# iKrishneel/fcn_object_detector

Measured on AMD Instinct MI355X. Metric: frames/sec forward 448x448 @1 GPU; train imgs/sec @1/2/4/8 GPUs, higher is better.
Workload: dtype f32; 1 GPU; configs[1]: single-GPU forward, DetectNet GoogLeNet conv stack + coverage/bbox heads (graph of models/deploy.prototxt), batch=1, 448x448, random-init weights; global_batch=1, parallelism=replicas x1, frames_in_flight=4

## Files before the change

### fcn_object_detector_amd/engine.py

```python
from __future__ import annotations

import ctypes as C
import os
import threading
from collections import namedtuple
from dataclasses import dataclass, field
from typing import Callable, Dict, List, Optional, Sequence, Tuple, Union

import numpy as np

from . import lib as L
from . import storage as S
from . import tune as T
from .netspec import Layer, NetSpec, bn_global_stats, crop_window, interp_size, is_rectangular, kernel_stride_pad, layer_dilation, layer_geometry
from .storage import _r4, _ra, ip_pack_bank, ip_unpack_bank

F32 = np.float32


def graphs_enabled() -> bool:
    return os.environ.get("FCN_NO_GRAPH", "0") in ("", "0")


_replica_ctx = threading.local()
# ... 74 lines not shown
    @property
    def bytes(self) -> float:
        return 4.0 * (self.n * self.cin * self.h * self.w + self.n * self.cout * self.oh * self.ow + self.cout * self.cin * self.kh * self.kw + self.cout)

    def swapped(self) -> "RectGeom":
        return self._replace(cin=self.cout, h=self.oh, w=self.ow, cout=self.cin, oh=self.h, ow=self.w)


def rconv_desc(x: "Blob", y: "Blob", g: RectGeom, w: Optional[int] = None, bias: Optional[int] = None, flags: int = 0) -> L.RConvDesc:
    d = L.RConvDesc()
    d.x, d.w, d.bias, d.y = x.ptr, w, bias, y.buf.ptr
    d.N, d.H, d.W, d.Cin, d.x_cstride = g.n, g.h, g.w, g.cin, x.cstride
    d.Cout, d.kh, d.kw, d.pad_h, d.pad_w, d.stride_h, d.stride_w, d.OH, d.OW = g.cout, g.kh, g.kw, g.ph, g.pw, g.sh, g.sw, g.oh, g.ow
    d.y_cstride, d.y_coffset = y.cstride, y.coffset
    d.flags, d.dilation = flags, g.d
    return d


class DwGeom(namedtuple("DwGeom", "n c h w oh ow kh kw sh sw ph pw d")):
    __slots__ = ()

    @property
    def flops(self) -> float:
        return 2.0 * self.n * self.oh * self.ow * self.c * self.kh * self.kw

    @property
    def bytes(self) -> float:
        return 4.0 * (self.n * self.h * self.w * self.c + self.n * self.oh * self.ow * self.c + self.kh * self.kw * self.c + self.c)


# ... 158 lines not shown
    return ranges_hit(later.reads, earlier.writes) or ranges_hit(later.writes, earlier.writes) or ranges_hit(later.writes, earlier.reads)


def task_levels(tasks: Sequence[Task], group_convs: bool = True) -> List[int]:
    levels: List[int] = []
    for i, ti in enumerate(tasks):
        levels.append(max([levels[j] + 1 for j in range(i) if task_waits(ti, tasks[j])], default=0) if group_convs else i)
    return levels


def task_floats(tasks: Sequence[Task], levels: Sequence[int], i: int) -> bool:
    return not any(levels[j] == levels[i] + 1 and task_waits(tj, tasks[i]) for j, tj in enumerate(tasks) if j != i)


class Engine:

    def __init__(self, spec: NetSpec, data_shapes: Optional[Dict[str, Tuple[int, ...]]] = None,
                 params: Optional[Dict[str, List[np.ndarray]]] = None, device: int = 0,
                 fuse: bool = True, group_convs: bool = True, autotune: bool = True, dtype: str = "f32",
                 tune_from: Optional["Engine"] = None, tune_max_lds_kb: Optional[int] = None,
                 share_params: Optional["Engine"] = None, score_outputs: bool = False, replica: Optional[int] = None):
        if dtype not in ("f32", "f16"):
            raise ValueError("dtype must be 'f32' or 'f16'")
        if share_params is not None and (dtype != "f32" or share_params.f16):
            raise NotImplementedError("share_params: only between float32 engines (a half-float engine packs its weights differently)")
        self._share_from = share_params
        self.shared_layers: set = set()
        self.score_outputs = bool(score_outputs)
        self.score_acc: Dict[str, DeviceBuffer] = {}
        self.graph_score: Optional[int] = None
# ... 16 lines not shown
        yes = C.c_int(0)
        L.call("fcn_stream_is_prioritized", self.stream, C.byref(yes))
        self.stream_prioritized = bool(yes.value)
        self.lock = threading.RLock()
        self.shapes = spec.infer(data_shapes)
        self.blobs: Dict[str, Blob] = {}
        self.params_host: Dict[str, List[np.ndarray]] = {}
        self.params_dev: Dict[str, List[DevView]] = {}
        self.ops: List[Op] = []
        self.graph_io: Optional[int] = None
        self.graph_core: Optional[int] = None
        self._staging: Dict[str, DeviceBuffer] = {}
        self._keep: List[object] = []
        self._conv_layer_meta: Dict[str, dict] = {}
        self._group_workspaces: List[DeviceBuffer] = []
        self.aux_dev: Dict[str, DeviceBuffer] = {}
        self._bn_chains: Dict[str, BnChain] = {}
        self._bn_ws_bytes = 0
        self._bn_ws: Optional[DeviceBuffer] = None
        self._lazy_blob_ops: Dict[str, List[Op]] = {}
        self.loss_blobs: Dict[str, float] = {}
        self.device_fed: set = set()
        self.dropout_seed = 0
        self.dropout_index_offset = 0
        self.inputs = spec.data_tops()
        self.outputs = [b for b in spec.output_blobs() if b in self.shapes]
        max_lds = int(tune_max_lds_kb if tune_max_lds_kb is not None else os.environ.get("FCN_TUNE_MAX_LDS_KB", "160")) * 1024
        self.tuner = T.Tuner(self.stream, T.key_suffix(self.shapes.get(self.inputs[0], ()) if self.inputs else None, self.f16, max_lds),
                             spec.phase == "TEST", max_lds, tune_from._chosen_cfgs if tune_from is not None else None)
        self._plan_buffers()
# ... 63 lines not shown
            self.param_segs[(seg.layer, seg.index)] = seg
            self.params_dev.setdefault(seg.layer, []).append(DevView(self.param_flat.ptr + 4 * seg.offset, seg.nbytes))
        for l in self.spec.param_layers():
            if l.name not in self.shared_layers:
                self._upload_params(l)

    def _folded_shift(self, l: Layer) -> float:
        return next((sh for t, sh in self._half_inputs.values() if t == l.bottoms[0]), 0.0) if l.type == "Convolution" else 0.0

    def _upload_params(self, l: Layer) -> None:
        if l.name in self.shared_layers:
            raise RuntimeError("layer %s reads the parameters of another engine (share_params): set them there" % l.name)
        packed = [S.pack(self.param_segs[(l.name, i)], h, self._folded_shift(l) if i == 0 else 0.0) for i, h in enumerate(self.params_host[l.name])]
        for arr, dev in zip(packed, self.params_dev[l.name]):
            L.call("fcn_memcpy_h2d_async", dev.ptr, arr.ctypes.data, arr.nbytes, None)
        L.call("fcn_device_sync")

    def set_params(self, layer: str, blobs: Sequence[np.ndarray]) -> None:
        lay = next(l for l in self.spec.layers if l.name == layer)
        if layer in self.shared_layers:
            raise RuntimeError("layer %s reads the parameters of another engine (share_params): set them there" % layer)
        shapes = self.spec.param_shapes[layer]
        self.params_host[layer] = [np.ascontiguousarray(b, dtype=F32).reshape(s).copy() for b, s in zip(blobs, shapes)]
        self._upload_params(lay)

    def read_param(self, layer: str, index: int) -> np.ndarray:
        with self.lock:
            v = self.params_dev[layer][index]
            raw = np.empty(v.nbytes, np.uint8)
            L.call("fcn_memcpy_d2h_async", raw.ctypes.data, v.ptr, raw.nbytes, self.stream)
# ... 218 lines not shown
            read = l.bottoms[:1] if t == "Crop" else l.bottoms
            tasks.append(OpTask(l, ops, reads=[self._range(b) for b in read], writes=[self._range(tp) for tp in l.tops],
                                pool_desc=self._fusable_pool_desc(l)))
        return tasks

    def _build_ops(self) -> None:
        tasks = self._collect_tasks()
        if self._bn_ws_bytes:
            self._bn_ws = DeviceBuffer(self._bn_ws_bytes, zero=False)
        if self.fuse and self.spec.phase == "TEST" and os.environ.get("FCN_FUSE_POOL_LRN", "1") != "0":
            tasks = self._fuse_pool_lrn(tasks)
        levels = task_levels(tasks, self.group_convs)
        if self.autotune and self.group_convs and self.fuse and not self.f16 and self.spec.phase == "TEST" and os.environ.get("FCN_LEVEL_MOVE", "1") != "0":
            self.tuner.move_floaters(tasks, levels)
        tail = self._plan_tail(tasks, levels)
        order = sorted(range(len(tasks)), key=lambda i: (levels[i], 1 if isinstance(tasks[i], ConvTask) else 0, i))
        pending: List[ConvTask] = []
        pending_pools: List[OpTask] = []
        pending_dconvs: List[OpTask] = []
        pending_rconvs: List[OpTask] = []
        cur = None
        for i in order:
            if levels[i] != cur:
                self._emit_dconvs(pending_dconvs)
                self._emit_rconvs(pending_rconvs)
                self._emit_convs(pending, pending_pools, tail)
                pending, pending_dconvs, pending_rconvs, cur = [], [], [], levels[i]
            if tail is not None and any(tasks[i] is ht for ht in tail["heads"]):
                continue
            if isinstance(tasks[i], ConvTask):
                pending.append(tasks[i])
            elif tasks[i].pool_desc is not None and self.fuse and self.group_convs:
                pending_pools.append(tasks[i])
            elif tasks[i].dconv is not None:
                pending_dconvs.append(tasks[i])
            elif tasks[i].rconv is not None:
                pending_rconvs.append(tasks[i])
            else:
                self.ops.extend(tasks[i].ops)
        self._emit_dconvs(pending_dconvs)
        self._emit_rconvs(pending_rconvs)
        self._emit_convs(pending, pending_pools, tail)
        self.levels = max(levels) + 1 if levels else 0
        if self.score_outputs:
            self._emit_score_ops()

    def _dconv_task(self, li: int, l: Layer, skip: set) -> OpTask:
        dil = layer_dilation(l)
        if self.f16:
            raise NotImplementedError("f16 engine: Convolution %s with dilation %d has no half-float kernel" % (l.name, dil))
        if self._conv_groups(l) > 1:
            raise NotImplementedError("Convolution %s: group %d together with dilation %d" % (l.name, self._conv_groups(l), dil))
        g = self._geom(l)
        xb, yb = self.blobs[l.bottoms[0]], self.blobs[l.tops[0]]
        if xb.coffset % 4 or xb.cstride % 4:
            raise NotImplementedError("dilated Convolution %s: input view is not 16-byte aligned" % l.name)
        relu = self._relu_after(li, l, skip)
        self._conv_layer_meta[l.name] = dict(relu=relu, sigmoid_top=None)
        pd = self.params_dev[l.name]
        d = dconv_desc(xb, yb, g, dil, pd[0].ptr, pd[1].ptr if len(pd) > 1 else None, L.CONV_RELU if relu else 0)
# ... 997 lines not shown
            for ws in getattr(self, "_group_workspaces", []):
                if ws.ptr:
                    lib.fcn_conv2d_group_release(ws.ptr)
                    ws.free()
            self._group_workspaces = []
            self.ops = []
            self.tuner.release()

    def __del__(self):
        try:
            self.close()
        except Exception:
            pass


class ForwardPipeline:

    def __init__(self, make_spec: Callable[[], NetSpec], params: Optional[Dict[str, List[np.ndarray]]] = None, device: int = 0, depth: int = 4,
                 max_lds_kb: Optional[int] = 36, **engine_kw):
        if depth < 1:
            raise ValueError("depth must be at least 1")
        self.engines: List[Engine] = []
        if os.environ.get("FCN_PIPE_LDS_KB"):
            max_lds_kb = int(os.environ["FCN_PIPE_LDS_KB"]) or None
        if max_lds_kb is not None:
            engine_kw.setdefault("tune_max_lds_kb", max_lds_kb)
        for i in range(depth):
            self.engines.append(Engine(make_spec(), params=params, device=device, tune_from=self.engines[0] if i else None, replica=i,
                                       **engine_kw))
        self._pending: List[Engine] = []
        self._next = 0

    @property
    def depth(self) -> int:
        return len(self.engines)

    def submit(self, inputs: Dict[str, np.ndarray]) -> None:
        if len(self._pending) >= len(self.engines):
            raise RuntimeError("ForwardPipeline: %d frames already in flight, collect() one first" % len(self._pending))
        eng = self.engines[self._next]
        self._next = (self._next + 1) % len(self.engines)
        for nm, arr in inputs.items():
            eng.host_array(nm)[...] = arr
        eng.forward_begin()
        self._pending.append(eng)

# ... 74 lines not shown
```

### fcn_object_detector_amd/lib.py

```python
from __future__ import annotations

import ctypes as C
import os
import threading
from typing import Optional

_HERE = os.path.dirname(os.path.abspath(__file__))
LIB_PATH = os.environ.get("FCN_LIB_PATH") or os.path.join(_HERE, "libfcnhip.so")


class FcnLibraryError(RuntimeError):
    pass


class FcnError(RuntimeError):
    def __init__(self, code: int, msg: str):
        super().__init__("libfcnhip error %d: %s" % (code, msg))
        self.code = code


class ConvDesc(C.Structure):
    _fields_ = [
        ("x", C.c_void_p), ("w", C.c_void_p), ("bias", C.c_void_p), ("y", C.c_void_p), ("y2", C.c_void_p),
        ("N", C.c_int32), ("H", C.c_int32), ("W", C.c_int32), ("Cin", C.c_int32), ("x_cstride", C.c_int32),
# ... 44 lines not shown
                ("total_tiles", C.c_int32)]


class RConvDesc(C.Structure):
    _fields_ = [
        ("x", C.c_void_p), ("w", C.c_void_p), ("bias", C.c_void_p), ("y", C.c_void_p), ("y2", C.c_void_p),
        ("N", C.c_int32), ("H", C.c_int32), ("W", C.c_int32), ("Cin", C.c_int32), ("x_cstride", C.c_int32),
        ("Cout", C.c_int32), ("kh", C.c_int32), ("kw", C.c_int32), ("pad_h", C.c_int32), ("pad_w", C.c_int32),
        ("stride_h", C.c_int32), ("stride_w", C.c_int32), ("OH", C.c_int32), ("OW", C.c_int32),
        ("y_cstride", C.c_int32), ("y_coffset", C.c_int32), ("y2_cstride", C.c_int32), ("y2_coffset", C.c_int32),
        ("flags", C.c_int32), ("dilation", C.c_int32),
    ]


class RConvPlan(C.Structure):
    _fields_ = [("d_probs", C.c_void_p), ("n", C.c_int32), ("cfg", C.c_int32), ("grid_x", C.c_int32), ("grid_y", C.c_int32),
                ("total_tiles", C.c_int32)]


class DwConvDesc(C.Structure):
    _fields_ = [
        ("x", C.c_void_p), ("w", C.c_void_p), ("bias", C.c_void_p), ("y", C.c_void_p), ("y2", C.c_void_p),
        ("N", C.c_int32), ("H", C.c_int32), ("W", C.c_int32), ("C", C.c_int32), ("x_cstride", C.c_int32),
        ("kh", C.c_int32), ("kw", C.c_int32), ("pad_h", C.c_int32), ("pad_w", C.c_int32),
        ("stride_h", C.c_int32), ("stride_w", C.c_int32), ("OH", C.c_int32), ("OW", C.c_int32),
        ("y_cstride", C.c_int32), ("y_coffset", C.c_int32), ("y2_cstride", C.c_int32), ("y2_coffset", C.c_int32),
        ("flags", C.c_int32), ("dilation", C.c_int32),
    ]


# ... 190 lines not shown
    "fcn_tconv_bank_floats": (_sz, [_i, _i, _i, _i]),
    "fcn_tconv_bank_pack_f32": (_i, [_vp, _vp, _i, _i, _i, _i, _i, _vp]),
    "fcn_channel_sum_f32": (_i, [_vp, _vp, _i, _i, _i, _i, _vp]),
    "fcn_dconv2d_num_configs": (_i, []),
    "fcn_dconv2d_workspace_bytes": (_sz, [C.POINTER(DConvDesc), _i]),
    "fcn_dconv2d_prepare": (_i, [C.POINTER(DConvDesc), _i, _vp, _i, C.POINTER(DConvPlan)]),
    "fcn_dconv2d_f32": (_i, [C.POINTER(DConvPlan), _vp]),
    "fcn_dconv2d_wgrad_workspace_floats": (_sz, [C.POINTER(DConvDesc)]),
    "fcn_dconv2d_wgrad_f32": (_i, [C.POINTER(DConvDesc), _vp, _vp, _vp, _vp]),
    "fcn_rconv2d_num_configs": (_i, []),
    "fcn_rconv2d_workspace_bytes": (_sz, [C.POINTER(RConvDesc), _i]),
    "fcn_rconv2d_prepare": (_i, [C.POINTER(RConvDesc), _i, _vp, _i, C.POINTER(RConvPlan)]),
    "fcn_rconv2d_f32": (_i, [C.POINTER(RConvPlan), _vp]),
    "fcn_rconv2d_wgrad_workspace_floats": (_sz, [C.POINTER(RConvDesc)]),
    "fcn_rconv2d_wgrad_f32": (_i, [C.POINTER(RConvDesc), _vp, _vp, _vp, _vp]),
    "fcn_dwconv2d_num_configs": (_i, []),
    "fcn_dwconv2d_fwd_f32": (_i, [C.POINTER(DwConvDesc), _i, _vp]),
    "fcn_dwconv2d_fwd_f16": (_i, [C.POINTER(DwConvDesc), _i, _vp]),
    "fcn_dwconv2d_dgrad_f32": (_i, [C.POINTER(DwConvDesc), _i, _vp]),
    "fcn_dwconv2d_wgrad_workspace_floats": (_sz, [C.POINTER(DwConvDesc), _i]),
    "fcn_dwconv2d_wgrad_f32": (_i, [C.POINTER(DwConvDesc), _vp, _vp, _vp, _i, _vp]),
    "fcn_crop_fwd_f32": (_i, [_vp, _vp] + [_i] * 12 + [_vp]),
    "fcn_crop_fwd_f16": (_i, [_vp, _vp] + [_i] * 12 + [_vp]),
    "fcn_crop_bwd_f32": (_i, [_vp, _vp] + [_i] * 13 + [_vp]),
    "fcn_interp_fwd_f32": (_i, [_vp, _vp] + [_i] * 12 + [_vp]),
    "fcn_interp_fwd_f16": (_i, [_vp, _vp] + [_i] * 13 + [_vp]),
    "fcn_interp_bwd_f32": (_i, [_vp, _vp] + [_i] * 13 + [_vp]),
    "fcn_inner_product_workspace_bytes": (_sz, [_i, _i, _i]),
    "fcn_inner_product_fwd_workspace_bytes": (_sz, [_i, _i, _i, _i]),
    "fcn_inner_product_fwd_f32": (_i, [_vp, _i, _vp, _vp, _vp] + [_i] * 6 + [_vp, _vp]),
# ... 72 lines not shown
```

### fcn_object_detector_amd/storage.py

```python
from __future__ import annotations

from dataclasses import dataclass
from typing import Dict, List, Optional, Sequence, Set, Tuple

import numpy as np

from .netspec import Layer, NetSpec, as_nchw

F32 = np.float32


def _r4(c: int) -> int:
    return (c + 3) // 4 * 4


def _ra(c: int, esize: int) -> int:
    eps = 16 // esize
    return (c + eps - 1) // eps * eps


def blob_nchw(shape: Sequence[int], rows: bool) -> Optional[Tuple[int, int, int, int]]:
    if rows and len(shape) == 1:
        return (shape[0], 1, 1, 1)
    return as_nchw(shape)
# ... 217 lines not shown
                elif f16:
                    raise NotImplementedError("f16 engine: layer type Deconvolution with group 1 (%s) has no half-float kernel" % l.name)
                else:
                    kind, shape = DECONV, (c, kh, kw, _r4(cog))
            elif i == 0 and l.type not in ("BatchNorm", "Scale"):
                raise NotImplementedError(l.type)
            count = int(np.prod(shape))
            lr, decay = float(l.lr_mult[i] if i < len(l.lr_mult) else 1.0), float(l.decay_mult[i] if i < len(l.decay_mult) else 1.0)
            if l.type == "BatchNorm":
                lr = decay = 0.0
            segs.append(ParamSeg(l.name, i, kind, off, count, shape, host_shape, lr, decay, count * esize, esize, bottom))
            off += _r4((count * esize + 3) // 4)
    return segs, off


def conv_groups(l: Layer, cout: int, cin_g: int, esize: int) -> int:
    g = int(l.sub("convolution_param").get("group", 1))
    if g == 1:
        return 1
    eps = 16 // esize
    if g < 1 or cout % g:
        raise ValueError("Convolution %s: group %d does not divide num_output %d" % (l.name, g, cout))
    if cin_g % eps or (cout // g) % eps:
        raise NotImplementedError("grouped Convolution %s: group %d leaves %d input and %d output channels per group, not whole 16-byte "
                                  "segments (%d %s)%s" % (l.name, g, cin_g, cout // g, eps, "floats" if esize == 4 else "halves",
                                                          ": depthwise convolution has no kernel here for a NetSpec built without "
                                                          "depthwise=True (caffe.Net and the solvers pass it; type DepthwiseConvolution "
                                                          "needs no keyword)" if cin_g == 1 else ""))
    return g

# ... 45 lines not shown
```

### fcn_object_detector_amd/train.py

```python
from __future__ import annotations

import ctypes as C
import os
import math
from typing import Callable, Dict, List, Optional, Sequence, Tuple

import numpy as np

from . import lib as L
from . import proto
from . import storage as S
from .backward import BackwardPlanner
from .engine import Blob, DevView, DeviceBuffer, Engine, Op, PinnedArray, _r4, graphs_enabled
from .netspec import DATA_TYPES, Layer, NetSpec

F32 = np.float32


class SolverParams:

    KINDS = ("SGD", "NESTEROV", "ADAGRAD", "RMSPROP", "ADADELTA", "ADAM")
    POLICIES = ("fixed", "step", "exp", "inv", "multistep", "poly", "sigmoid")

    def __init__(self, msg: Optional[proto.Msg] = None, **kw):
# ... 79 lines not shown
            return b
        if p == "step":
            return b * self.gamma ** (it // self.stepsize)
        if p == "exp":
            return b * self.gamma ** it
        if p == "inv":
            return b * (1.0 + self.gamma * it) ** (-self.power)
        if p == "multistep":
            return b * self.gamma ** sum(1 for v in self.stepvalue if v <= it)
        if p == "poly":
            return b * (1.0 - float(it) / self.max_iter) ** self.power
        return b / (1.0 + math.exp(-self.gamma * (it - self.stepsize)))


class TrainEngine(Engine):

    def __init__(self, spec: NetSpec, data_shapes: Dict[str, Tuple[int, ...]], params=None, device: int = 0,
                 solver: Optional[SolverParams] = None, comm=None, autotune: bool = True):
        if spec.phase != "TRAIN":
            raise ValueError("TrainEngine needs a TRAIN-phase NetSpec")
        self.solver = solver or SolverParams()
        self.comm = comm
        self.grad_blobs: Dict[str, Blob] = {}
        self.bwd_ops: List[Op] = []
        self.iter = 0
        super().__init__(spec, data_shapes, params, device, fuse=True, group_convs=True, autotune=autotune)
        self._alloc_solver_state()
        self._build_backward()

    def _learns(self, l: Layer) -> bool:
# ... 452 lines not shown
```

### fcn_object_detector_amd/tune.py

```python
from __future__ import annotations

import ctypes as C
import json
import os
from typing import Callable, Dict, Iterable, List, NamedTuple, Optional, Sequence, Tuple

import numpy as np

from . import engine as E
from . import lib as L


def lower_quartile(samples: Sequence[float]) -> float:
    return float(np.percentile(samples, 25))


class Protocol(NamedTuple):
    warm: int
    reps: int
    evict: bool
    samples: int
    stat: Callable[[Sequence[float]], float]
    contenders: int
    margin: float
# ... 182 lines not shown
                return memo[sub]

            best, best_ms = None, 1e30
            for labels in set_partitions(n):
                ms = sum(cost(tuple(i for i in range(n) if labels[i] == g)) for g in sorted(set(labels)))
                if ms < best_ms - 1e-7:
                    best, best_ms = labels, ms
            return "".join(str(g) for g in best)

        choice = self.choose("cut|" + self.key("+".join(it.layer.name for it in chunk)), valid, search)
        groups: Dict[str, List[E.ConvTask]] = {}
        for it, g in zip(chunk, choice):
            groups.setdefault(g, []).append(it)
        return [groups[g] for g in sorted(groups)]

    def move_floaters(self, tasks: Sequence[object], levels: List[int]) -> None:
        for lv in range(max(levels, default=-1)):
            a_idx, b_idx = ([i for i, t in enumerate(tasks) if levels[i] == l2 and isinstance(t, E.ConvTask)] for l2 in (lv, lv + 1))
            if len(a_idx) < 2 or not b_idx or len(a_idx) > 8:
                continue
            fl = [i for i in a_idx if E.task_floats(tasks, levels, i)]
            if not fl or len(fl) > 3 or len(b_idx) + len(fl) > 8:
                continue

            def valid(code) -> bool:
                return isinstance(code, str) and len(code) == len(fl) and set(code) <= {"0", "1"} and (len(fl) < len(a_idx) or "0" in code)

            def search() -> str:
                pools = {l2: [t.pool_desc for j, t in enumerate(tasks) if levels[j] == l2 and isinstance(t, E.OpTask) and t.pool_desc is not None][:2]
                         for l2 in (lv, lv + 1)}
# ... 28 lines not shown
```

### include/fcnhip.h

```cpp
#ifndef FCNHIP_H_
#define FCNHIP_H_

#include <stddef.h>
#include <stdint.h>

#ifdef __cplusplus
extern "C" {
#endif

#define FCN_ABI_VERSION 1

#define FCN_E_ARG       1
#define FCN_E_ALIGN     2
#define FCN_E_UNSUPPORTED 3
#define FCN_E_STATE     4
#define FCN_E_CAPACITY  5

typedef void* fcn_stream_t;
typedef void* fcn_event_t;
typedef void* fcn_graph_t;
typedef void* fcn_comm_t;

int  fcn_abi_version(void);
const char* fcn_last_error_string(void);
// ... 344 lines not shown
} fcn_rconv_desc;
typedef struct fcn_rconv_plan {
    void*   d_probs;
    int32_t n;
    int32_t cfg;
    int32_t grid_x, grid_y;
    int32_t total_tiles;
} fcn_rconv_plan;
int    fcn_rconv2d_num_configs(void);
size_t fcn_rconv2d_workspace_bytes(const fcn_rconv_desc* h_descs, int n);
int    fcn_rconv2d_prepare(const fcn_rconv_desc* h_descs, int n, void* d_workspace, int cfg_request, fcn_rconv_plan* h_out);
int    fcn_rconv2d_f32(const fcn_rconv_plan* h_plan, fcn_stream_t s);
size_t fcn_rconv2d_wgrad_workspace_floats(const fcn_rconv_desc* h_d);
int    fcn_rconv2d_wgrad_f32(const fcn_rconv_desc* h_d, float* dw, float* db, float* d_workspace, fcn_stream_t s);

typedef struct fcn_dwconv_desc {
    void*        x;
    const float* w;
    const float* bias;
    void*        y;
    float*       y2;
    int32_t N, H, W, C, x_cstride;
    int32_t kh, kw, pad_h, pad_w, stride_h, stride_w, OH, OW;
    int32_t y_cstride, y_coffset, y2_cstride, y2_coffset;
    int32_t flags;
    int32_t dilation;
} fcn_dwconv_desc;
int    fcn_dwconv2d_num_configs(void);
int    fcn_dwconv2d_fwd_f32(const fcn_dwconv_desc* h_d, int cfg_request, fcn_stream_t s);
int    fcn_dwconv2d_fwd_f16(const fcn_dwconv_desc* h_d, int cfg_request, fcn_stream_t s);
// ... 58 lines not shown
```

Before: 4576 frames/s.

## Add Winograd F(2x2,3x3) MFMA conv kernel for eligible inference 3x3 convs

Adds a Winograd F(2,3) convolution kernel for stride-1, pad-1 3x3 float32 convolutions. The input transform is done in-register with DPP lane permutes, the 16 transformed-domain GEMMs run on f32 MFMA, and the output transform plus bias and ReLU are fused into the epilogue. Filter banks are pre-transformed on the host when weights are uploaded. Placement is decided per layer by timing the layer with and without the Winograd kernel, and a multi-replica 'flight' mode is also tuned; the path is limited to inference. The aim is fewer multiplies on the 3x3 convolutions, at the cost of extra filter memory, tuning time and slightly different float rounding.

```diff
diff --git a/fcn_object_detector_amd/csrc/wconv.hip b/fcn_object_detector_amd/csrc/wconv.hip
--- /dev/null
+++ b/fcn_object_detector_amd/csrc/wconv.hip
@@ -0,0 +1,298 @@
+#include "conv_common.h"
+
+#include <vector>
+
+namespace fcn {
+namespace {
+
+constexpr int WC_TILES = 32;
+constexpr int WC_BN = 32;
+constexpr int WC_BK = 8;
+constexpr int WC_POS = 16;
+constexpr int WC_THREADS = 256;
+constexpr int WC_STAGE = WC_POS * 32 * WC_BK;
+constexpr int WC_CONFIGS = 1;
+
+struct WConvP {
+    const float* x;
+    const float* u;
+    const float* bias;
+    float* y;
+    int N, H, W, Cin, x_cstride, Cout, OH, OW, y_cstride, y_coffset, flags;
+    int TH, TW, tiles, nblk_n, nchunk;
+    unsigned tw_magic, th_magic;
+};
+
+template <int S0, int S1, int S2, int S3>
+__device__ __forceinline__ float quad_perm(float v) {
+    return __builtin_bit_cast(float, __builtin_amdgcn_update_dpp(0, __builtin_bit_cast(int, v), S0 | (S1 << 2) | (S2 << 4) | (S3 << 6), 0xf, 0xf, false));
+}
+
+__global__ __launch_bounds__(WC_THREADS) void wconv_f32_kernel(const WConvP* __restrict__ probs) {
+    const WConvP& p = probs[blockIdx.z];
+    const int tblk = blockIdx.x, nblk = blockIdx.y;
+    if (tblk * WC_TILES >= p.tiles || nblk >= p.nblk_n) return;
+
+    __shared__ __attribute__((aligned(16))) float smem[4 * WC_STAGE];
+    float* const sV = smem;
+    float* const sU = smem + 2 * WC_STAGE;
+
+    const int tid = threadIdx.x, lane = tid & 63, wave = tid >> 6;
+    const int lj = tid & 3, lq = (tid >> 2) & 1, lt = tid >> 3;
+    int l_off[4] = {0, 0, 0, 0};
+    bool l_ok[4] = {false, false, false, false};
+    {
+        const int t = tblk * WC_TILES + lt;
+        if (t < p.tiles) {
+            const int q = fast_div(t, p.tw_magic), tx = t - q * p.TW;
+            const int n = fast_div(q, p.th_magic), ty = q - n * p.TH;
+            const int ix = 2 * tx - 1 + lj;
+#pragma unroll
+            for (int i = 0; i < 4; ++i) {
+                const int iy = 2 * ty - 1 + i;
+                l_ok[i] = (unsigned)ix < (unsigned)p.W && (unsigned)iy < (unsigned)p.H;
+                l_off[i] = l_ok[i] ? ((n * p.H + iy) * p.W + ix) * p.x_cstride : 0;
+            }
+        }
+    }
+    const float* const ubase = p.u + (size_t)nblk * p.nchunk * WC_STAGE + tid * 4;
+    const int sign_q = lj == 1 ? 0 : (int)0x80000000u;
+
+    v4f regX[4], regU[4];
+    auto fetch = [&](int c) {
+        const float* us = ubase + (size_t)c * WC_STAGE;
+#pragma unroll
+        for (int r = 0; r < 4; ++r) regU[r] = *(const v4f*)(us + r * (WC_THREADS * 4));
+        const int ci = c * WC_BK + lq * 4;
+#pragma unroll
+        for (int i = 0; i < 4; ++i) {
+            regX[i] = v4f{0.f, 0.f, 0.f, 0.f};
+            if (l_ok[i] && ci < p.Cin) {
+                regX[i] = *(const v4f*)(p.x + l_off[i] + ci);
+                if (ci + 1 >= p.Cin) regX[i][1] = 0.f;
+                if (ci + 2 >= p.Cin) regX[i][2] = 0.f;
+                if (ci + 3 >= p.Cin) regX[i][3] = 0.f;
+            }
+        }
+    };
+    auto stage = [&](int buf) {
+        float* dv = sV + buf * WC_STAGE + ((lt + lj) & 31) * WC_BK + lq * 4;
+        float* du = sU + buf * WC_STAGE + tid * 4;
+#pragma unroll
+        for (int r = 0; r < 4; ++r) *(v4f*)(du + r * (WC_THREADS * 4)) = regU[r];
+        v4f t[4];
+        t[0] = regX[0] - regX[2];
+        t[1] = regX[1] + regX[2];
+        t[2] = regX[2] - regX[1];
+        t[3] = regX[1] - regX[3];
+#pragma unroll
+        for (int i = 0; i < 4; ++i) {
+            v4f v;
+#pragma unroll
+            for (int e = 0; e < 4; ++e) {
+                const float a = quad_perm<0, 1, 2, 1>(t[i][e]);
+                const float b = quad_perm<2, 2, 1, 3>(t[i][e]);
+                v[e] = a + __builtin_bit_cast(float, __builtin_bit_cast(int, b) ^ sign_q);
+            }
+            *(v4f*)(dv + (i * 4 + lj) * (32 * WC_BK)) = v;
+        }
+    };
+
+    const int fr = lane & 31, fh = lane >> 5;
+    const int frag = (wave * 4 * 32 + fr) * WC_BK + fh * 4;
+    int fragv[4];
+#pragma unroll
+    for (int pp = 0; pp < 4; ++pp) fragv[pp] = ((wave * 4 + pp) * 32 + ((fr + pp) & 31)) * WC_BK + fh * 4;
+    f32x16 acc[4];
+#pragma unroll
+    for (int pp = 0; pp < 4; ++pp)
+#pragma unroll
+        for (int e = 0; e < 16; ++e) acc[pp][e] = 0.f;
+
+    fetch(0);
+#pragma unroll 1
+    for (int it = 0; it < p.nchunk; ++it) {
+        const int buf = it & 1;
+        stage(buf);
+        if (it + 1 < p.nchunk) fetch(it + 1);
+        __syncthreads();
+        v4f uf[4], vf[4];
+#pragma unroll
+        for (int pp = 0; pp < 4; ++pp) {
+            uf[pp] = *(const v4f*)(sU + buf * WC_STAGE + frag + pp * (32 * WC_BK));
+            vf[pp] = *(const v4f*)(sV + buf * WC_STAGE + fragv[pp]);
+        }
+#pragma unroll
+        for (int e = 0; e < 4; ++e)
+#pragma unroll
+            for (int pp = 0; pp < 4; ++pp) acc[pp] = __builtin_amdgcn_mfma_f32_32x32x2f32(uf[pp][e], vf[pp][e], acc[pp], 0, 0, 0);
+    }
+
+    __syncthreads();
+#pragma unroll
+    for (int pp = 0; pp < 4; ++pp)
+#pragma unroll
+        for (int r = 0; r < 16; ++r)
+            smem[((wave * 4 + pp) * 32 + (r & 3) + 8 * (r >> 2) + 4 * fh) * 32 + fr] = acc[pp][r];
+    __syncthreads();
+
+    const int et = tid & 31, eq = tid >> 5;
+    const int t = tblk * WC_TILES + et;
+    const int co = nblk * WC_BN + eq * 4;
+    if (t >= p.tiles || co >= p.Cout) return;
+    v4f s[2][4];
+#pragma unroll
+    for (int j = 0; j < 4; ++j)
+#pragma unroll
+        for (int e = 0; e < 4; ++e) {
+            const float m0 = smem[((0 * 4 + j) * 32 + eq * 4 + e) * 32 + et], m1 = smem[((1 * 4 + j) * 32 + eq * 4 + e) * 32 + et];
+            const float m2 = smem[((2 * 4 + j) * 32 + eq * 4 + e) * 32 + et], m3 = smem[((3 * 4 + j) * 32 + eq * 4 + e) * 32 + et];
+            s[0][j][e] = (m0 + m1) + m2;
+            s[1][j][e] = (m1 - m2) - m3;
+        }
+    const int q = fast_div(t, p.tw_magic), tx = t - q * p.TW;
+    const int n = fast_div(q, p.th_magic), ty = q - n * p.TH;
+    const bool do_relu = (p.flags & FCN_CONV_RELU) != 0;
+    const bool vec_ok = ((p.y_cstride | p.y_coffset) & 3) == 0 && ((unsigned)(size_t)p.y & 15) == 0 && co + 3 < p.Cout;
+    v4f b4 = {0.f, 0.f, 0.f, 0.f};
+    if (p.bias)
+#pragma unroll
+        for (int e = 0; e < 4; ++e)
+            if (co + e < p.Cout) b4[e] = p.bias[co + e];
+#pragma unroll
+    for (int dy = 0; dy < 2; ++dy)
+#pragma unroll
+        for (int dx = 0; dx < 2; ++dx) {
+            const int oy = 2 * ty + dy, ox = 2 * tx + dx;
+            if (oy >= p.OH || ox >= p.OW) continue;
+            v4f v = dx == 0 ? (s[dy][0] + s[dy][1]) + s[dy][2] : (s[dy][1] - s[dy][2]) - s[dy][3];
+            v += b4;
+            if (do_relu)
+#pragma unroll
+                for (int e = 0; e < 4; ++e) v[e] = fmaxf(v[e], 0.f);
+            float* dst = p.y + (size_t)((n * p.OH + oy) * p.OW + ox) * p.y_cstride + p.y_coffset + co;
+            if (vec_ok) {
+                *(v4f*)dst = v;
+            } else {
+#pragma unroll
+                for (int e = 0; e < 4; ++e)
+                    if (co + e < p.Cout) dst[e] = v[e];
+            }
+        }
+}
+
+int validate(const fcn_wconv_desc& d) {
+    FCN_REQUIRE(d.x && d.y && d.u, FCN_E_ARG, "wconv: null x/u/y");
+    FCN_REQUIRE(d.N > 0 && d.H > 0 && d.W > 0 && d.Cin > 0 && d.Cout > 0, FCN_E_ARG, "wconv: non-positive extent");
+    FCN_REQUIRE(d.kh == 3 && d.kw == 3, FCN_E_UNSUPPORTED, "wconv: kernel window %dx%d is not 3x3", d.kh, d.kw);
+    FCN_REQUIRE(d.stride_h == 1 && d.stride_w == 1, FCN_E_UNSUPPORTED, "wconv: stride %dx%d is not 1", d.stride_h, d.stride_w);
+    FCN_REQUIRE(d.pad_h == 1 && d.pad_w == 1, FCN_E_UNSUPPORTED, "wconv: pad %dx%d is not 1", d.pad_h, d.pad_w);
+    FCN_REQUIRE(d.dilation == 1, FCN_E_UNSUPPORTED, "wconv: dilation %d is not 1", d.dilation);
+    FCN_REQUIRE((d.flags & ~FCN_CONV_RELU) == 0, FCN_E_UNSUPPORTED,
+                "wconv: flags 0x%x outside FCN_CONV_RELU (float32 only; no FCN_CONV_F16 / SIGMOID2 / ACCUM / MASK)", d.flags);
+    FCN_REQUIRE(d.Cin % 4 == 0, FCN_E_ALIGN, "wconv: Cin (%d) must be a multiple of 4", d.Cin);
+    FCN_REQUIRE(d.x_cstride % 4 == 0 && d.x_cstride >= d.Cin, FCN_E_ALIGN, "wconv: x_cstride (%d) must be a multiple of 4 holding Cin (%d)", d.x_cstride,
+                d.Cin);
+    FCN_REQUIRE(((uintptr_t)d.x & 15) == 0 && ((uintptr_t)d.u & 15) == 0, FCN_E_ALIGN, "wconv: x / u must be 16-byte aligned");
+    FCN_REQUIRE(((uintptr_t)d.y & 3) == 0 && (!d.bias || ((uintptr_t)d.bias & 3) == 0), FCN_E_ALIGN, "wconv: y / bias must be 4-byte aligned");
+    FCN_REQUIRE(d.OH == d.H && d.OW == d.W, FCN_E_ARG, "wconv: OH/OW (%d,%d) is not H/W (%d,%d)", d.OH, d.OW, d.H, d.W);
+    FCN_REQUIRE(d.y_coffset >= 0 && d.y_cstride >= d.y_coffset + d.Cout, FCN_E_ARG, "wconv: output slice exceeds y_cstride");
+    const long long tiles = (long long)d.N * ((d.OH + 1) / 2) * ((d.OW + 1) / 2);
+    FCN_REQUIRE((long long)d.N * d.H * d.W * d.x_cstride < (1ll << 31) && (long long)d.N * d.OH * d.OW * d.y_cstride < (1ll << 31) &&
+                    (tiles + WC_TILES) * (((d.OH > d.OW ? d.OH : d.OW) + 1) / 2) < (1ll << 32),
+                FCN_E_UNSUPPORTED, "wconv: tensor too large for 32-bit element offsets");
+    return 0;
+}
+
+unsigned magic_of(int d) { return d <= 1 ? 0u : (unsigned)(((1ull << 32) + (unsigned)d - 1) / (unsigned)d); }
+
+}
+}
+
+using namespace fcn;
+
+extern "C" {
+
+int fcn_wconv2d_num_configs(void) { return WC_CONFIGS; }
+
+size_t fcn_wconv2d_workspace_bytes(const fcn_wconv_desc* h_descs, int n) {
+    (void)h_descs;
+    return n > 0 ? (size_t)n * sizeof(WConvP) : 0;
+}
+
+size_t fcn_wconv2d_bank_floats(int Cout, int Cin) {
+    if (Cout <= 0 || Cin <= 0) return 0;
+    return (size_t)((Cout + WC_BN - 1) / WC_BN) * ((Cin + WC_BK - 1) / WC_BK) * WC_STAGE;
+}
+
+int fcn_wconv2d_transform_filters(const float* h_w, int Cout, int Cin, int w_cstride, float* h_u) {
+    FCN_REQUIRE(h_w && h_u, FCN_E_ARG, "wconv transform: null bank");
+    FCN_REQUIRE(Cout > 0 && Cin > 0 && w_cstride >= Cin, FCN_E_ARG, "wconv transform: Cout (%d) / Cin (%d) / row stride (%d)", Cout, Cin, w_cstride);
+    const int nchunk = (Cin + WC_BK - 1) / WC_BK;
+    const size_t total = fcn_wconv2d_bank_floats(Cout, Cin);
+    for (size_t i = 0; i < total; ++i) h_u[i] = 0.f;
+    static const double G[4][3] = {{1.0, 0.0, 0.0}, {0.5, 0.5, 0.5}, {0.5, -0.5, 0.5}, {0.0, 0.0, 1.0}};
+    for (int co = 0; co < Cout; ++co) {
+        const float* g = h_w + (size_t)co * 9 * w_cstride;
+        float* ub = h_u + (size_t)(co / WC_BN) * nchunk * WC_STAGE + (size_t)(co % WC_BN) * WC_BK;
+        for (int ci = 0; ci < Cin; ++ci) {
+            double gg[4][3];
+            for (int i = 0; i < 4; ++i)
+                for (int q = 0; q < 3; ++q)
+                    gg[i][q] = G[i][0] * g[(0 * 3 + q) * w_cstride + ci] + G[i][1] * g[(1 * 3 + q) * w_cstride + ci] + G[i][2] * g[(2 * 3 + q) * w_cstride + ci];
+            float* uc = ub + (size_t)(ci / WC_BK) * WC_STAGE + ci % WC_BK;
+            for (int i = 0; i < 4; ++i)
+                for (int j = 0; j < 4; ++j)
+                    uc[(i * 4 + j) * (32 * WC_BK)] = (float)(gg[i][0] * G[j][0] + gg[i][1] * G[j][1] + gg[i][2] * G[j][2]);
+        }
+    }
+    return 0;
+}
+
+int fcn_wconv2d_prepare(const fcn_wconv_desc* h_descs, int n, void* d_workspace, int cfg_request, fcn_wconv_plan* h_out) {
+    FCN_REQUIRE(h_descs && h_out && n > 0, FCN_E_ARG, "wconv prepare: null descriptors / plan or n <= 0");
+    FCN_REQUIRE(n <= 65535, FCN_E_UNSUPPORTED, "wconv prepare: more than 65535 problems");
+    FCN_REQUIRE(cfg_request >= -1 && cfg_request < WC_CONFIGS, FCN_E_ARG, "wconv prepare: unknown configuration %d", cfg_request);
+    long long gx = 0, gy = 0, total = 0;
+    std::vector<WConvP> ps((size_t)n);
+    for (int i = 0; i < n; ++i) {
+        const fcn_wconv_desc& d = h_descs[i];
+        const int rc = validate(d);
+        if (rc) return rc;
+        WConvP& p = ps[(size_t)i];
+        p.x = d.x; p.u = d.u; p.bias = d.bias; p.y = d.y;
+        p.N = d.N; p.H = d.H; p.W = d.W; p.Cin = d.Cin; p.x_cstride = d.x_cstride; p.Cout = d.Cout; p.OH = d.OH; p.OW = d.OW;
+        p.y_cstride = d.y_cstride; p.y_coffset = d.y_coffset; p.flags = d.flags;
+        p.TH = (d.OH + 1) / 2; p.TW = (d.OW + 1) / 2;
+        p.tiles = d.N * p.TH * p.TW;
+        p.nblk_n = (d.Cout + WC_BN - 1) / WC_BN;
+        p.nchunk = (d.Cin + WC_BK - 1) / WC_BK;
+        p.tw_magic = magic_of(p.TW); p.th_magic = magic_of(p.TH);
+        const long long bx = (p.tiles + WC_TILES - 1) / WC_TILES;
+        gx = bx > gx ? bx : gx;
+        gy = p.nblk_n > gy ? p.nblk_n : gy;
+        total += bx * p.nblk_n;
+    }
+    FCN_REQUIRE(gx < (1ll << 31) && gy <= 65535 && total < (1ll << 31), FCN_E_UNSUPPORTED, "wconv prepare: too many tiles for one launch");
+    FCN_REQUIRE(d_workspace, FCN_E_ARG, "wconv prepare: null workspace");
+    FCN_HIP(hipMemcpy(d_workspace, ps.data(), ps.size() * sizeof(WConvP), hipMemcpyHostToDevice));
+    h_out->d_probs = d_workspace;
+    h_out->n = n;
+    h_out->cfg = 0;
+    h_out->grid_x = (int32_t)gx;
+    h_out->grid_y = (int32_t)gy;
+    h_out->total_tiles = (int32_t)total;
+    return 0;
+}
+
+int fcn_wconv2d_f32(const fcn_wconv_plan* h_plan, fcn_stream_t s) {
+    const fcn_wconv_plan plan = h_plan ? *h_plan : fcn_wconv_plan{};
+    FCN_REQUIRE(plan.d_probs && plan.n > 0 && plan.grid_x > 0 && plan.grid_y > 0 && plan.grid_y <= 65535 && plan.n <= 65535 && plan.cfg == 0, FCN_E_ARG,
+                "wconv: the plan was not filled by fcn_wconv2d_prepare");
+    hipLaunchKernelGGL(wconv_f32_kernel, dim3((unsigned)plan.grid_x, (unsigned)plan.grid_y, (unsigned)plan.n), dim3(WC_THREADS), 0, as_stream(s),
+                       (const WConvP*)plan.d_probs);
+    FCN_LAUNCH_CHECK("wconv_f32_kernel");
+    return 0;
+}
+
+}
diff --git a/fcn_object_detector_amd/engine.py b/fcn_object_detector_amd/engine.py
--- a/fcn_object_detector_amd/engine.py
+++ b/fcn_object_detector_amd/engine.py
@@ -112,6 +112,15 @@
     d.Cout, d.kh, d.kw, d.pad_h, d.pad_w, d.stride_h, d.stride_w, d.OH, d.OW = g.cout, g.kh, g.kw, g.ph, g.pw, g.sh, g.sw, g.oh, g.ow
     d.y_cstride, d.y_coffset = y.cstride, y.coffset
     d.flags, d.dilation = flags, g.d
+    return d
+
+
+def wconv_desc(x: "Blob", y: "Blob", g: ConvGeom, u: Optional[int] = None, bias: Optional[int] = None, flags: int = 0) -> L.WConvDesc:
+    d = L.WConvDesc()
+    d.x, d.u, d.bias, d.y, d.y2 = x.ptr, u, bias, y.buf.ptr, None
+    d.N, d.H, d.W, d.Cin, d.x_cstride = g.n, g.h, g.w, g.cin, x.cstride
+    d.Cout, d.kh, d.kw, d.pad_h, d.pad_w, d.stride_h, d.stride_w, d.OH, d.OW = g.cout, g.k, g.k, g.pad, g.pad, g.s, g.s, g.oh, g.ow
+    d.y_cstride, d.y_coffset, d.flags, d.dilation = y.cstride, y.coffset, flags, 1
     return d
 
 
@@ -300,6 +309,8 @@
 
 
 class Engine:
+
+    winograd = True
 
     def __init__(self, spec: NetSpec, data_shapes: Optional[Dict[str, Tuple[int, ...]]] = None,
                  params: Optional[Dict[str, List[np.ndarray]]] = None, device: int = 0,
@@ -346,6 +357,8 @@
         self._keep: List[object] = []
         self._conv_layer_meta: Dict[str, dict] = {}
         self._group_workspaces: List[DeviceBuffer] = []
+        self._wconv_banks: Dict[str, DeviceBuffer] = {}
+        self.wconv_keys: Dict[str, str] = {}
         self.aux_dev: Dict[str, DeviceBuffer] = {}
         self._bn_chains: Dict[str, BnChain] = {}
         self._bn_ws_bytes = 0
@@ -439,6 +452,13 @@
         packed = [S.pack(self.param_segs[(l.name, i)], h, self._folded_shift(l) if i == 0 else 0.0) for i, h in enumerate(self.params_host[l.name])]
         for arr, dev in zip(packed, self.params_dev[l.name]):
             L.call("fcn_memcpy_h2d_async", dev.ptr, arr.ctypes.data, arr.nbytes, None)
+        L.call("fcn_device_sync")
+        if l.name in getattr(self, "_wconv_banks", ()):
+            self._upload_wconv_bank(l.name)
+
+    def _upload_wconv_bank(self, layer: str) -> None:
+        u = S.winograd_pack(self.params_host[layer][0])
+        L.call("fcn_memcpy_h2d_async", self._wconv_banks[layer].ptr, u.ctypes.data, u.nbytes, None)
         L.call("fcn_device_sync")
 
     def set_params(self, layer: str, blobs: Sequence[np.ndarray]) -> None:
@@ -687,6 +707,7 @@
         if self.autotune and self.group_convs and self.fuse and not self.f16 and self.spec.phase == "TEST" and os.environ.get("FCN_LEVEL_MOVE", "1") != "0":
             self.tuner.move_floaters(tasks, levels)
         tail = self._plan_tail(tasks, levels)
+        self._place_wconvs(tasks, levels, tail["producers"] if tail is not None else ())
         order = sorted(range(len(tasks)), key=lambda i: (levels[i], 1 if isinstance(tasks[i], ConvTask) else 0, i))
         pending: List[ConvTask] = []
         pending_pools: List[OpTask] = []
@@ -717,6 +738,56 @@
         self.levels = max(levels) + 1 if levels else 0
         if self.score_outputs:
             self._emit_score_ops()
+
+    def _wconv_eligible(self, t: Task) -> bool:
+        if not (self.winograd and self.autotune and self.fuse and self.group_convs and not self.f16 and self.spec.phase == "TEST"):
+            return False
+        if not isinstance(t, ConvTask) or t.layer.name in self.shared_layers or os.environ.get("FCN_WINOGRAD", "") == "0":
+            return False
+        d = t.desc
+        return (S.winograd_eligible(t.layer, self.spec.param_shapes[t.layer.name][0]) and (d.flags & ~L.CONV_RELU) == 0 and d.in_shift == 0.0
+                and d.Cin % 4 == 0 and self.blobs[t.layer.tops[0]].esize == 4)
+
+    def _wconv_task(self, t: ConvTask) -> OpTask:
+        lib = L.load()
+        l, g = t.layer, self._geom(t.layer)
+        if l.name not in self._wconv_banks:
+            self._wconv_banks[l.name] = DeviceBuffer(4 * S.winograd_bank_floats(g.cout, g.cin), zero=False)
+            self._upload_wconv_bank(l.name)
+        pd = self.params_dev[l.name]
+        d = wconv_desc(self.blobs[l.bottoms[0]], self.blobs[l.tops[0]], g, self._wconv_banks[l.name].ptr, pd[1].ptr if len(pd) > 1 else None,
+                       t.desc.flags & L.CONV_RELU)
+        arr = (L.WConvDesc * 1)(d)
+        ws = DeviceBuffer(int(lib.fcn_wconv2d_workspace_bytes(arr, 1)), zero=False)
+        plan = L.WConvPlan()
+        L.call("fcn_wconv2d_prepare", arr, 1, ws.ptr, -1, C.byref(plan))
+        self._keep.extend([arr, ws, plan])
+        op = Op("conv_winograd", "%s [F(2x2,3x3) %dwg, flops as direct]" % (l.name, plan.total_tiles),
+                lambda st, p=plan: L.check(lib.fcn_wconv2d_f32(C.byref(p), st)), t.flops, t.bytes)
+        return OpTask(l, [op], reads=t.reads, writes=t.writes)
+
+    def _place_wconvs(self, tasks: List[Task], levels: List[int], keep: Sequence[int] = ()) -> None:
+        for i, t in enumerate(tasks):
+            if id(t) in keep or not self._wconv_eligible(t):
+                continue
+            key = "wino|" + self.tuner.key(t.layer.name)
+            self.wconv_keys[t.layer.name] = key
+            valid = lambda v: type(v) is int and v in (0, 1)
+            if os.environ.get("FCN_WINOGRAD", "") != "1" and not any(k is not None and valid(k.get(key)) for k in (self.tuner.tune_from, self.tuner.cache)):
+                continue
+            made: List[OpTask] = []
+
+            def search(i=i, t=t, made=made) -> int:
+                made.append(self._wconv_task(t))
+                level = [j for j, tj in enumerate(tasks) if levels[j] == levels[i] and isinstance(tj, ConvTask)]
+                pools = [tj.pool_desc for j, tj in enumerate(tasks) if levels[j] == levels[i] and isinstance(tj, OpTask) and tj.pool_desc is not None][:2]
+                return self.tuner.wconv_pays(made[0].ops[0], [tasks[j].desc for j in level], [tasks[j].desc for j in level if j != i],
+                                             pools if len(level) <= 8 else [])
+
+            if self.tuner.choose(key, valid, search):
+                tasks[i] = made[0] if made else self._wconv_task(t)
+            elif t.layer.name in self._wconv_banks:
+                self._wconv_banks.pop(t.layer.name).free()
 
     def _dconv_task(self, li: int, l: Layer, skip: set) -> OpTask:
         dil = layer_dilation(l)
@@ -1744,6 +1815,12 @@
             pass
 
 
+class _TunePlan:
+
+    def __init__(self, chosen: Dict[str, object]):
+        self._chosen_cfgs = chosen
+
+
 class ForwardPipeline:
 
     def __init__(self, make_spec: Callable[[], NetSpec], params: Optional[Dict[str, List[np.ndarray]]] = None, device: int = 0, depth: int = 4,
@@ -1755,11 +1832,58 @@
             max_lds_kb = int(os.environ["FCN_PIPE_LDS_KB"]) or None
         if max_lds_kb is not None:
             engine_kw.setdefault("tune_max_lds_kb", max_lds_kb)
-        for i in range(depth):
-            self.engines.append(Engine(make_spec(), params=params, device=device, tune_from=self.engines[0] if i else None, replica=i,
-                                       **engine_kw))
+        def build(plan: Optional[object]) -> List[Engine]:
+            engines: List[Engine] = []
+            for i in range(depth):
+                engines.append(Engine(make_spec(), params=params, device=device, tune_from=engines[0] if i else plan, replica=i, **engine_kw))
+            return engines
+
+        self.engines = build(None)
+        self.winograd_mode = self._place_wconvs_in_flight(build) if depth > 1 and self.engines[0].wconv_keys else None
         self._pending: List[Engine] = []
         self._next = 0
+
+    def _place_wconvs_in_flight(self, build: Callable[[Optional[object]], List[Engine]]) -> str:
+        import time
+        lib = L.load()
+        first = self.engines[0]
+        keys = first.wconv_keys
+        solo = {k: int(first.tuner.chosen.get(k, 0)) for k in keys.values()}
+        self.winograd_lone_ms = getattr(first.tuner, "wconv_ms", {})
+        plans = {"off": {k: 0 for k in solo}, "solo": solo, "all": {k: 1 for k in solo}}
+
+        def replan(mode: str) -> None:
+            if plans[mode] == {k: int(self.engines[0].tuner.chosen.get(k, 0)) for k in solo}:
+                return
+            chosen = dict(first.tuner.chosen)
+            chosen.update(plans[mode])
+            self.close()
+            self.engines = []
+            self.engines = build(_TunePlan(chosen))
+
+        def search() -> str:
+            iters = int(os.environ.get("FCN_WINOGRAD_FLIGHT_ITERS", "120"))
+            ms: Dict[str, float] = {}
+            for mode in ("off", "solo", "all"):
+                same = next((m for m in ms if plans[m] == plans[mode]), None)
+                if same is not None:
+                    ms[mode] = ms[same]
+                    continue
+                replan(mode)
+                self._run_resident(self.engines, iters, lib, time)
+                ms[mode] = min(self._run_resident(self.engines, iters, lib, time) for _ in range(3))
+            self.winograd_flight_ms = {m: 1e3 * v / iters for m, v in ms.items()}
+            best = min(("solo", "all"), key=lambda m: ms[m])
+            return best if ms[best] < 0.99 * ms["off"] else "off"
+
+        key, valid = "winoflight|" + first.tuner.key("+".join(keys)) + "|d%d" % len(self.engines), lambda v: v in ("off", "solo", "all")
+        if os.environ.get("FCN_WINOGRAD", "") != "1" and not any(k is not None and valid(k.get(key)) for k in (first.tuner.tune_from, first.tuner.cache)):
+            return "solo"
+        mode = first.tuner.choose(key, valid, search)
+        replan(mode)
+        if self.engines[0] is not first:
+            self.engines[0].tuner.chosen.update({k: v for k, v in first.tuner.chosen.items() if k.startswith("winoflight|")})
+        return mode
 
     @property
     def depth(self) -> int:
diff --git a/fcn_object_detector_amd/lib.py b/fcn_object_detector_amd/lib.py
--- a/fcn_object_detector_amd/lib.py
+++ b/fcn_object_detector_amd/lib.py
@@ -82,6 +82,22 @@
 
 
 class RConvPlan(C.Structure):
+    _fields_ = [("d_probs", C.c_void_p), ("n", C.c_int32), ("cfg", C.c_int32), ("grid_x", C.c_int32), ("grid_y", C.c_int32),
+                ("total_tiles", C.c_int32)]
+
+
+class WConvDesc(C.Structure):
+    _fields_ = [
+        ("x", C.c_void_p), ("u", C.c_void_p), ("bias", C.c_void_p), ("y", C.c_void_p), ("y2", C.c_void_p),
+        ("N", C.c_int32), ("H", C.c_int32), ("W", C.c_int32), ("Cin", C.c_int32), ("x_cstride", C.c_int32),
+        ("Cout", C.c_int32), ("kh", C.c_int32), ("kw", C.c_int32), ("pad_h", C.c_int32), ("pad_w", C.c_int32),
+        ("stride_h", C.c_int32), ("stride_w", C.c_int32), ("OH", C.c_int32), ("OW", C.c_int32),
+        ("y_cstride", C.c_int32), ("y_coffset", C.c_int32), ("y2_cstride", C.c_int32), ("y2_coffset", C.c_int32),
+        ("flags", C.c_int32), ("dilation", C.c_int32),
+    ]
+
+
+class WConvPlan(C.Structure):
     _fields_ = [("d_probs", C.c_void_p), ("n", C.c_int32), ("cfg", C.c_int32), ("grid_x", C.c_int32), ("grid_y", C.c_int32),
                 ("total_tiles", C.c_int32)]
 
@@ -302,6 +318,12 @@
     "fcn_rconv2d_f32": (_i, [C.POINTER(RConvPlan), _vp]),
     "fcn_rconv2d_wgrad_workspace_floats": (_sz, [C.POINTER(RConvDesc)]),
     "fcn_rconv2d_wgrad_f32": (_i, [C.POINTER(RConvDesc), _vp, _vp, _vp, _vp]),
+    "fcn_wconv2d_num_configs": (_i, []),
+    "fcn_wconv2d_workspace_bytes": (_sz, [C.POINTER(WConvDesc), _i]),
+    "fcn_wconv2d_bank_floats": (_sz, [_i, _i]),
+    "fcn_wconv2d_transform_filters": (_i, [_vp, _i, _i, _i, _vp]),
+    "fcn_wconv2d_prepare": (_i, [C.POINTER(WConvDesc), _i, _vp, _i, C.POINTER(WConvPlan)]),
+    "fcn_wconv2d_f32": (_i, [C.POINTER(WConvPlan), _vp]),
     "fcn_dwconv2d_num_configs": (_i, []),
     "fcn_dwconv2d_fwd_f32": (_i, [C.POINTER(DwConvDesc), _i, _vp]),
     "fcn_dwconv2d_fwd_f16": (_i, [C.POINTER(DwConvDesc), _i, _vp]),
diff --git a/fcn_object_detector_amd/storage.py b/fcn_object_detector_amd/storage.py
--- a/fcn_object_detector_amd/storage.py
+++ b/fcn_object_detector_amd/storage.py
@@ -255,6 +255,35 @@
     return segs, off
 
 
+WINOGRAD_BN, WINOGRAD_BK, WINOGRAD_STAGE = 32, 8, 16 * 32 * 8
+_WINOGRAD_G = np.array([[1.0, 0.0, 0.0], [0.5, 0.5, 0.5], [0.5, -0.5, 0.5], [0.0, 0.0, 1.0]], np.float64)
+
+
+def winograd_bank_floats(cout: int, cin: int) -> int:
+    return -(-cout // WINOGRAD_BN) * -(-cin // WINOGRAD_BK) * WINOGRAD_STAGE
+
+
+def winograd_pack(w: np.ndarray) -> np.ndarray:
+    a = np.asarray(w, np.float64)
+    cout, cin, kh, kw = a.shape
+    if (kh, kw) != (3, 3):
+        raise ValueError("winograd_pack: a %dx%d window is not 3x3" % (kh, kw))
+    G = _WINOGRAD_G
+    gg = (G[:, 0, None, None, None] * a[:, :, 0][None] + G[:, 1, None, None, None] * a[:, :, 1][None]) + G[:, 2, None, None, None] * a[:, :, 2][None]
+    u = (gg[:, None, :, :, 0] * G[None, :, 0, None, None] + gg[:, None, :, :, 1] * G[None, :, 1, None, None]) + gg[:, None, :, :, 2] * G[None, :, 2, None, None]
+    nb, nc = -(-cout // WINOGRAD_BN), -(-cin // WINOGRAD_BK)
+    full = np.zeros((16, nb * WINOGRAD_BN, nc * WINOGRAD_BK), F32)
+    full[:, :cout, :cin] = u.reshape(16, cout, cin).astype(F32)
+    return np.ascontiguousarray(full.reshape(16, nb, WINOGRAD_BN, nc, WINOGRAD_BK).transpose(1, 3, 0, 2, 4)).reshape(-1)
+
+
+def winograd_eligible(l: Layer, param_shape: Sequence[int]) -> bool:
+    from .netspec import is_rectangular, kernel_stride_pad, layer_dilation
+    if l.type != "Convolution" or is_rectangular(l) or layer_dilation(l) != 1 or int(l.sub("convolution_param").get("group", 1)) != 1:
+        return False
+    return tuple(kernel_stride_pad(l.sub("convolution_param"))) == (3, 1, 1) and len(param_shape) == 4 and int(param_shape[1]) % 4 == 0
+
+
 def conv_groups(l: Layer, cout: int, cin_g: int, esize: int) -> int:
     g = int(l.sub("convolution_param").get("group", 1))
     if g == 1:
diff --git a/fcn_object_detector_amd/train.py b/fcn_object_detector_amd/train.py
--- a/fcn_object_detector_amd/train.py
+++ b/fcn_object_detector_amd/train.py
@@ -117,6 +117,8 @@
 
 
 class TrainEngine(Engine):
+
+    winograd = False
 
     def __init__(self, spec: NetSpec, data_shapes: Dict[str, Tuple[int, ...]], params=None, device: int = 0,
                  solver: Optional[SolverParams] = None, comm=None, autotune: bool = True):
diff --git a/fcn_object_detector_amd/tune.py b/fcn_object_detector_amd/tune.py
--- a/fcn_object_detector_amd/tune.py
+++ b/fcn_object_detector_amd/tune.py
@@ -220,6 +220,19 @@
             groups.setdefault(g, []).append(it)
         return [groups[g] for g in sorted(groups)]
 
+    def wconv_pays(self, op: "E.Op", level: Sequence[L.ConvDesc], rest: Sequence[L.ConvDesc], pools: Sequence[L.PoolDesc]) -> int:
+        cold = self.cold and os.environ.get("FCN_TUNE_COLD", "1") != "0"
+        p = COLD if cold else WARM
+        base = min(self._subset_ms(level, pools) for _ in range(2))
+        alone = min(self.fastest([0], lambda cfg: True, lambda: op.run(self.stream), p, False)[1] for _ in range(2))
+        without = 0.0
+        if rest:
+            floor = min(self.fastest([0], lambda cfg: True, lambda: None, p, False)[1] for _ in range(2))
+            without = min(self._subset_ms(rest, pools) for _ in range(2)) - floor
+        self.wconv_ms = getattr(self, "wconv_ms", {})
+        self.wconv_ms[op.name] = dict(level_ms=base, winograd_ms=alone, rest_ms=without)
+        return 1 if alone + without < float(os.environ.get("FCN_MOVE_MARGIN", "0.99")) * base else 0
+
     def move_floaters(self, tasks: Sequence[object], levels: List[int]) -> None:
         for lv in range(max(levels, default=-1)):
             a_idx, b_idx = ([i for i, t in enumerate(tasks) if levels[i] == l2 and isinstance(t, E.ConvTask)] for l2 in (lv, lv + 1))
diff --git a/include/fcnhip.h b/include/fcnhip.h
--- a/include/fcnhip.h
+++ b/include/fcnhip.h
@@ -382,6 +382,32 @@
 size_t fcn_rconv2d_wgrad_workspace_floats(const fcn_rconv_desc* h_d);
 int    fcn_rconv2d_wgrad_f32(const fcn_rconv_desc* h_d, float* dw, float* db, float* d_workspace, fcn_stream_t s);
 
+typedef struct fcn_wconv_desc {
+    const float* x;
+    const float* u;
+    const float* bias;
+    float*       y;
+    float*       y2;
+    int32_t N, H, W, Cin, x_cstride;
+    int32_t Cout, kh, kw, pad_h, pad_w, stride_h, stride_w, OH, OW;
+    int32_t y_cstride, y_coffset, y2_cstride, y2_coffset;
+    int32_t flags;
+    int32_t dilation;
+} fcn_wconv_desc;
+typedef struct fcn_wconv_plan {
+    void*   d_probs;
+    int32_t n;
+    int32_t cfg;
+    int32_t grid_x, grid_y;
+    int32_t total_tiles;
+} fcn_wconv_plan;
+int    fcn_wconv2d_num_configs(void);
+size_t fcn_wconv2d_workspace_bytes(const fcn_wconv_desc* h_descs, int n);
+size_t fcn_wconv2d_bank_floats(int Cout, int Cin);
+int    fcn_wconv2d_transform_filters(const float* h_w, int Cout, int Cin, int w_cstride, float* h_u);
+int    fcn_wconv2d_prepare(const fcn_wconv_desc* h_descs, int n, void* d_workspace, int cfg_request, fcn_wconv_plan* h_out);
+int    fcn_wconv2d_f32(const fcn_wconv_plan* h_plan, fcn_stream_t s);
+
 typedef struct fcn_dwconv_desc {
     void*        x;
     const float* w;
```

Result: no change. 4553 frames/s (-0.5%).
